# mjmyt/drone_path_planning_python

Hardware: AMD Instinct MI355X
Metric: minimum-snap trajectories/sec (N drones × M segments, order 7) at 1/2/4/8 MI355X (higher is better)
Workload: dtype f64

## Files before the change

### drone_path_planning_python_amd/csrc/msnap_collide.hip

```cpp
#include <math.h>

#include "msnap_internal.h"
#include "msnap_collide.h"
#include "msnap_wave.h"

namespace msnap {


struct CollideGeom {
  int R, ro, Cn, S;
  int Rp;
  int os, oe;
  int sym;
  int n_rb;
  int upw;
  int upw_tail;
  long long split;
  int sparts;
  long long total;
  long long u_lo, u_n;
  int I_lo, I_hi;
  int part;
};

// ... 395 lines not shown
        const int e = threadIdx.x + u * kSelThreads;
        bv[u] = e < nG * 6 ? cu.colbox[e] : 0.0;
      }
#pragma unroll
      for (int u = 0; u < kStageGroups * 6 / kSelThreads; ++u) {
        const int e = threadIdx.x + u * kSelThreads;
        if (e < nG * 6) sBox[e] = bv[u];
      }
    }
    __syncthreads();
  }
  auto load_box = [&](int gq, double(&B)[6]) {
#pragma unroll
    for (int k = 0; k < 6; ++k) {
      if constexpr (kStage) B[k] = sBox[gq * 6 + k];
      else B[k] = cu.colbox[(size_t)gq * 6 + k];
    }
  };
  if ((int)blockIdx.x >= n_rb) {
    constexpr int NW = kSelThreads / kWave, NS = kSelGroups * kSelTrips;
    __shared__ int gsum[NS * NW + 1];
    __shared__ int gbase, gtot;
    const int a0 = (blockIdx.x - n_rb) * kSelGroups, nG = (N + kColBlock - 1) / kColBlock;
    const int lane = threadIdx.x & (kWave - 1), w = threadIdx.x / kWave;
    unsigned long long kept = 0;
#pragma unroll
    for (int ai = 0; ai < kSelGroups; ++ai) {
      const int a = a0 + ai;
      double A[7], A6[6];
      load_box(a < nG ? a : nG - 1, A6);
#pragma unroll
      for (int k = 0; k < 6; ++k) A[k] = A6[k];
      A[6] = sCmax[a < nG ? a : nG - 1];
#pragma unroll
      for (int t = 0; t < kSelTrips; ++t) {
        bool keep = false;
        if (a + t * kSelThreads < nG) {
          const int b = a + t * kSelThreads + threadIdx.x, bc = b < nG ? b : nG - 1;
          double B6[6];
          load_box(bc, B6);
          const double lb2 = box_box_lb2(A, B6);
          keep = b < nG && (b == a || !((lb2 > A[6]) & (lb2 > sCmax[bc])));
        }
        const unsigned long long m = __ballot(keep);
        kept |= keep ? 1ull << (ai * kSelTrips + t) : 0ull;
        if (lane == 0) gsum[(ai * kSelTrips + t) * NW + w] = __popcll(m);
      }
    }
    __syncthreads();
    if (threadIdx.x < kWave) {
      int run = 0;
      for (int i0 = 0; i0 < NS * NW; i0 += kWave) {
        const int v = i0 + lane < NS * NW ? gsum[i0 + lane] : 0;
        int inc = v;
#pragma unroll
        for (int m = 1; m < kWave; m <<= 1) {
          const int o = __shfl_up(inc, m);
          inc += lane >= m ? o : 0;
        }
        if (i0 + lane < NS * NW) gsum[i0 + lane] = run + inc - v;
        run += __shfl(inc, kWave - 1);
      }
      if (lane == 0) {
        gbase = atomicAdd(&meta[kMetaGroups], run);
        gtot = run;
      }
    }
    __syncthreads();
    if (threadIdx.x < kSelGroups && a0 + (int)threadIdx.x < nG) {
      const int ai = threadIdx.x;
      const int s0 = gsum[ai * kSelTrips * NW], s1 = ai + 1 < kSelGroups ? gsum[(ai + 1) * kSelTrips * NW] : gtot;
      cg.astart[a0 + ai] = gbase + s0;
      cg.acnt[a0 + ai] = s1 - s0;
    }
#pragma unroll
    for (int ai = 0; ai < kSelGroups; ++ai)
#pragma unroll
      for (int t = 0; t < kSelTrips; ++t) {
        const bool keep = (kept >> (ai * kSelTrips + t)) & 1ull;
        const unsigned long long m = __ballot(keep);
        const int pos = gbase + gsum[(ai * kSelTrips + t) * NW + w] + __popcll(m & ((1ull << lane) - 1ull));
        if (keep && pos < cg.cap) {
          const int a = a0 + ai, b = a + t * kSelThreads + threadIdx.x;
          cg.glist[pos] = (a << 16) | b;
          if (b != a) cg.blist[(size_t)b * cg.nG + a] = pos + 1;
        }
      }
    return;
  }
  constexpr int GPB = kRowBlock / kColBlock;
  constexpr int NW = kSelThreads / kWave;
  __shared__ int wsum[kSelTrips][NW];
  __shared__ int sStart;
  __shared__ double sRow[GPB][8];
  __shared__ double sAll[8];
  const int I = blockIdx.x, lane = threadIdx.x & (kWave - 1), w = threadIdx.x / kWave;
  const int nsh = (N - I * kRowBlock + kColBlock - 1) / kColBlock;
  const int ng = nsh < GPB ? nsh : GPB;
  if (threadIdx.x < 7 * GPB) {
    const int q = threadIdx.x / 7, k = threadIdx.x % 7;
    if (q < ng) sRow[q][k] = k < 6 ? (kStage ? sBox[(I * GPB + q) * 6 + k] : cu.colbox[(size_t)(I * GPB + q) * 6 + k]) : sCmax[I * GPB + q];
  }
  __syncthreads();
  if (threadIdx.x < 7) {
    const int k = threadIdx.x;
    double v = sRow[0][k];
    for (int q = 1; q < ng; ++q) v = k < 3 ? fmin(v, sRow[q][k]) : fmax(v, sRow[q][k]);
    sAll[k] = v;
  }
  __syncthreads();
  unsigned long long mk[kSelTrips];
  bool keep[kSelTrips];
  double cbx[kSelTrips][6], cmx[kSelTrips];
#pragma unroll
  for (int t = 0; t < kSelTrips; ++t) {
    if (t * kSelThreads >= nsh) continue;
    const int k = t * kSelThreads + threadIdx.x, J = I * GPB + (k < nsh ? k : nsh - 1);
    load_box(J, cbx[t]);
    cmx[t] = sCmax[J];
  }
#pragma unroll
  for (int t = 0; t < kSelTrips; ++t) {
    const int k = t * kSelThreads + threadIdx.x;
    keep[t] = false;
    if (k < nsh) {
      keep[t] = true;
      if (k >= GPB) {
        const double cm = cmx[t];
        bool any = false;
        const double lb0 = box_box_lb2(sAll, cbx[t]);
        if (!((lb0 > sAll[6]) & (lb0 > cm))) {
          for (int q = 0; q < ng; ++q) {
            const double lb2 = box_box_lb2(sRow[q], cbx[t]);
            any |= !((lb2 > sRow[q][6]) & (lb2 > cm));
          }
        }
        keep[t] = any;
      }
    }
    mk[t] = __ballot(keep[t]);
    if (lane == 0) wsum[t][w] = __popcll(mk[t]);
  }
  __syncthreads();
  int all = 0, off[kSelTrips];
#pragma unroll
  for (int t = 0; t < kSelTrips; ++t) {
#pragma unroll
    for (int q = 0; q < NW; ++q) {
      if (q == w) off[t] = all;
      all += wsum[t][q];
    }
  }
  if (threadIdx.x == 0) {
    const int start = atomicAdd(&meta[kMetaTotal], all);
    sStart = start;
    meta[kMetaStart + I] = start;
    cnt[I] = all;
  }
  __syncthreads();
#pragma unroll
  for (int t = 0; t < kSelTrips; ++t)
    if (keep[t]) list[sStart + off[t] + __popcll(mk[t] & ((1ull << lane) - 1ull))] = (I << 16) | (t * kSelThreads + threadIdx.x);
}

__device__ __forceinline__ void
collide_span_list_body(const double *__restrict__ prow_t, const double *__restrict__ pcol, CollideGeom g,
                       double *__restrict__ part_d2, int32_t *__restrict__ part_j, double *__restrict__ cpart_d2,
                       int32_t *__restrict__ cpart_i, const int32_t *__restrict__ oid, const int32_t *__restrict__ list,
                       int sp_force, int slots, int32_t *__restrict__ meta) {
  constexpr int CB = kColBlock;
  __shared__ double sFold[CB * kWave];
  __shared__ int sFoldI[CB * kWave];
  const int lane = threadIdx.x;
  const int tot = meta[kMetaTotal];
  const CullSplit sp = cull_split(tot, slots, cull_nch(g.S), sp_force);
  if (blockIdx.x == 0 && lane == 0) {
    meta[kMetaParts] = sp.lo;
    meta[kMetaParts + 1] = sp.hi;
    meta[kMetaParts + 2] = sp.x;
  }
  const int items = sp.items(tot);
  const int xi = sp.x * sp.hi;
  auto share_of = [&](int it) { return it < xi ? it / sp.hi : sp.x + (it - xi) / sp.lo; };
  int it = blockIdx.x;
  int entry = it < items ? list[share_of(it)] : 0;
  while (it < items) {
    const int f = share_of(it);
    g.sparts = it < xi ? sp.hi : sp.lo;
    const int h = it - sp.item_of(f);
    const int I = entry >> 16, k = entry & 0xffff;
    const int nxt = it + gridDim.x;
    entry = nxt < items ? list[share_of(nxt)] : 0;
    const int crow = I * sp.hi + h;
    const int cj = I * kRowBlock + k * CB;
    const int ncols = g.Cn - cj < CB ? g.Cn - cj : CB;
    const bool two_sided = k >= kRowBlock / CB;
    RowSet rs;
#pragma unroll
    for (int rr = 0; rr < kRowsPerLane; ++rr) {
      const int raw = I * kRowBlock + rr * kWave + lane;
      rs.live[rr] = raw < g.R;
      rs.grow[rr] = rs.live[rr] ? raw : g.R - 1;
      rs.best[rr] = INFINITY;
      rs.bestj[rr] = -1;
    }
    const double *prowT = prow_t + (size_t)I * kRowBlock;
    if (ncols <= 2)
      collide_block<2, true>(g, prowT, pcol, cj, ncols, two_sided, rs, I, h, crow, lane, sFold, sFoldI, cpart_d2, cpart_i, oid);
    else if (ncols <= CB / 2)
      collide_block<CB / 2, true>(g, prowT, pcol, cj, ncols, two_sided, rs, I, h, crow, lane, sFold, sFoldI, cpart_d2, cpart_i, oid);
    else
      collide_block<CB, true>(g, prowT, pcol, cj, ncols, two_sided, rs, I, h, crow, lane, sFold, sFoldI, cpart_d2, cpart_i, oid);
#pragma unroll
    for (int rr = 0; rr < kRowsPerLane; ++rr) {
      part_d2[(size_t)it * kRowBlock + rr * kWave + lane] = rs.best[rr];
      part_j[(size_t)it * kRowBlock + rr * kWave + lane] = (rs.best[rr] == INFINITY) ? -1 : rs.bestj[rr];
    }
    it = nxt;
  }
}

constexpr int kGroupHalf = kColBlock / 2;
constexpr int kGroupLanes = kWave / 2;

constexpr int kFinishWaves = 4;
template <int kChunks>
__global__ void __launch_bounds__(kWave * kFinishWaves)
collide_finish_groups_kernel(int N, const int32_t *__restrict__ oid, const int32_t *__restrict__ meta, CullGroups cg,
                             double radius, double *__restrict__ min_dist, int32_t *__restrict__ partner,
                             int32_t *__restrict__ hit) {
  __shared__ int sItAll[kFinishWaves][kChunks * kWave];
  const int lane = threadIdx.x & (kWave - 1), w = __builtin_amdgcn_readfirstlane(threadIdx.x / kWave);
  int *sIt = sItAll[w];
  const int gq = blockIdx.x * kFinishWaves + w;
  if (gq >= cg.nG) return;
  int pl[kChunks];
#pragma unroll
  for (int c = 0; c < kChunks; ++c)
    pl[c] = (c * kWave < gq && c * kWave + lane < gq) ? cg.blist[(size_t)gq * cg.nG + c * kWave + lane] : 0;
  if (meta[kMetaGroups] > cg.cap) {
#pragma unroll
    for (int c = 0; c < kChunks; ++c)
      if (pl[c] > 0) cg.blist[(size_t)gq * cg.nG + c * kWave + lane] = 0;
    return;
  }
  const int nA = cg.acnt[gq], sA = cg.astart[gq];
  const int k = lane & (kColBlock - 1), e = lane >> 3;
  const int r = gq * kColBlock + k;
  const int out = r < N ? oid[r] : 0;
  int nB = 0;
#pragma unroll
  for (int c = 0; c < kChunks; ++c) {
    const unsigned long long m = __ballot(pl[c] > 0);
    if (pl[c] > 0) sIt[nB + __popcll(m & ((1ull << lane) - 1ull))] = pl[c] - 1;
    nB += __popcll(m);
  }
  __builtin_amdgcn_fence(__ATOMIC_RELEASE, "wavefront", "local");
  __builtin_amdgcn_wave_barrier();
  __builtin_amdgcn_fence(__ATOMIC_ACQUIRE, "wavefront", "local");
  double best = INFINITY;
  int bj = -1;
  constexpr int U = 8;
  for (int q0 = 0; q0 < nA + nB; q0 += U * (kWave / kColBlock)) {
    double d[U];
    int j[U];
#pragma unroll
    for (int u = 0; u < U; ++u) {
      const int q = q0 + u * (kWave / kColBlock) + e;
      d[u] = INFINITY;
      j[u] = -1;
      if (q < nA + nB) {
        const size_t slot = (q < nA ? (size_t)(sA + q) * 16 : (size_t)sIt[q - nA] * 16 + kColBlock) + k;
        d[u] = cg.cand_d2[slot];
        j[u] = cg.cand_j[slot];
      }
    }
#pragma unroll
    for (int u = 0; u < U; ++u)
      if (j[u] >= 0 && (bj < 0 || d[u] < best || (d[u] == best && j[u] < bj))) {
        best = d[u];
        bj = j[u];
      }
  }
#pragma unroll
  for (int m = kColBlock; m < kWave; m <<= 1) {
    const double o = shfl_xor_f64(best, m);
    const int oj = __shfl_xor(bj, m);
    if (oj >= 0 && (bj < 0 || o < best || (o == best && oj < bj))) {
      best = o;
      bj = oj;
    }
  }
  if (e == 0 && r < N) {
    const double dist = sqrt(bj >= 0 ? best : INFINITY);
    min_dist[out] = dist;
    partner[out] = bj;
    hit[out] = (dist < 2.0 * radius) ? 1 : 0;
  }
#pragma unroll
  for (int c = 0; c < kChunks; ++c)
    if (pl[c] > 0) cg.blist[(size_t)gq * cg.nG + c * kWave + lane] = 0;
}

constexpr int kGroupWaves = 4;
__global__ void __launch_bounds__(kWave, kGroupWaves)
collide_eval_groups_kernel(const double *__restrict__ pcol, int N, int S, const int32_t *__restrict__ oid,
                           const int32_t *__restrict__ meta, CullGroups cg, unsigned long long *__restrict__ hint) {
#pragma clang fp contract(off)
  const int lane = threadIdx.x;
  int tot = meta[kMetaGroups];
  if (blockIdx.x == 0 && lane == 0 && hint != nullptr)
    __hip_atomic_store(hint, cull_hint_pack(N, meta[kMetaTotal], tot), __ATOMIC_RELAXED, __HIP_MEMORY_SCOPE_SYSTEM);
  if (tot > cg.cap) tot = 0;
  const unsigned stride = (unsigned)S * 3u;
  const int per = (tot + 7) >> 3;
  auto item_of = [&](int v) { return (v >> 3) < per ? (v & 7) * per + (v >> 3) : tot; };
  int v = blockIdx.x, it = item_of(v);
  int entry = (it < tot && it < cg.cap) ? cg.glist[it] : 0;
  for (; (v >> 3) < per; v += gridDim.x, it = item_of(v)) {
    const int it_next = item_of(v + (int)gridDim.x);
    const int ent_raw = entry;
    entry = it_next < tot ? cg.glist[it_next] : 0;
    if (it >= tot) continue;
    const int ent = __builtin_amdgcn_readfirstlane(ent_raw);
    const int a = ent >> 16, b = ent & 0xffff;
    const bool diag = a == b;

    int lane_s = threadIdx.x;
    asm volatile("" : "+v"(lane_s));
    const int half = lane_s >> 5, ls = lane_s & (kGroupLanes - 1);
    double acc[kColBlock * kGroupHalf];
#pragma unroll
    for (int p = 0; p < kColBlock * kGroupHalf; ++p) acc[p] = INFINITY;
#pragma unroll 1
    for (int s0 = 0; s0 < S; s0 += kGroupLanes) {
      const int sq = s0 + ls < S ? s0 + ls : S - 1;
      const unsigned voff = (unsigned)sq * 24u;
      double cx[kGroupHalf], cy[kGroupHalf], cz[kGroupHalf];
#pragma unroll
      for (int c = 0; c < kGroupHalf; ++c) {
        const int d = b * kColBlock + half * kGroupHalf + c;
        const double *p = reinterpret_cast<const double *>(
            reinterpret_cast<const char *>(pcol + (size_t)(d < N ? d : N - 1) * stride) + (size_t)voff);
        cx[c] = p[0];
        cy[c] = p[1];
        cz[c] = p[2];
      }
      double rw[3][3];
      auto fetch = [&](int r, double(&dst)[3]) {
        const int d = a * kColBlock + r;
        const double *p = reinterpret_cast<const double *>(
            reinterpret_cast<const char *>(pcol + (size_t)(d < N ? d : N - 1) * stride) + (size_t)voff);
        dst[0] = p[0];
        dst[1] = p[1];
        dst[2] = p[2];
      };
      fetch(0, rw[0]);
      fetch(1, rw[1]);
#pragma unroll
      for (int r = 0; r < kColBlock; ++r) {
        if (r + 2 < kColBlock) fetch(r + 2, rw[(r + 2) % 3]);
        asm volatile("" ::: "memory");
        const double x = rw[r % 3][0], y = rw[r % 3][1], z = rw[r % 3][2];
#pragma unroll
        for (int c = 0; c < kGroupHalf; ++c) {
          const double dx = cx[c] - x, dy = cy[c] - y, dz = cz[c] - z;
          const double d2 = __builtin_fma(dz, dz, __builtin_fma(dy, dy, dx * dx));
          asm("v_min_f64 %0, %1, %0" : "+v"(acc[r * kGroupHalf + c]) : "v"(d2));
        }
      }
    }
#pragma unroll
    for (int n = 16, m = 16; n >= 1; n >>= 1, m >>= 1) {
      const bool up = (lane_s & m) != 0;
#pragma unroll
      for (int i = 0; i < n; ++i) {
        const double keep = up ? acc[i + n] : acc[i], send = up ? acc[i] : acc[i + n];
        acc[i] = __builtin_fmin(keep, __shfl_xor(send, m));
      }
    }
    double v = acc[0];
    int lane_c = threadIdx.x;
    asm volatile("" : "+v"(lane_c));
    const int pr = (lane_c & (kGroupLanes - 1)) >> 2, pc = lane_c & (kGroupHalf - 1), half_c = lane_c >> 5;
    const int ra = a * kColBlock + pr, cb = b * kColBlock + half_c * kGroupHalf + pc;
    const int oi = oid[ra < N ? ra : N - 1], oj = oid[cb < N ? cb : N - 1];
    if (ra >= N || cb >= N || (diag && ra == cb)) v = INFINITY;
    {
      double w = v;
      int wj = oj;
#pragma unroll
      for (int m = 1; m <= 32; m = (m == 2 ? 32 : m << 1)) {
        const double o = __shfl_xor(w, m);
        const int ojx = __shfl_xor(wj, m);
        const bool take = (o < w) | ((o == w) & (ojx < wj));
        w = take ? o : w;
        wj = take ? ojx : wj;
      }
      if ((lane & 35) == 0) {
        cg.cand_d2[(size_t)it * 16 + pr] = w;
        cg.cand_j[(size_t)it * 16 + pr] = w < INFINITY ? wj : -1;
      }
    }
    {
      double w = v;
      int wi = oi;
#pragma unroll
      for (int m = 4; m <= 16; m <<= 1) {
        const double o = __shfl_xor(w, m);
        const int oix = __shfl_xor(wi, m);
        const bool take = (o < w) | ((o == w) & (oix < wi));
        w = take ? o : w;
        wi = take ? oix : wi;
      }
      if ((lane_c & (kGroupLanes - 1)) < kGroupHalf) {
        const int k = kColBlock + half_c * kGroupHalf + pc;
        cg.cand_d2[(size_t)it * 16 + k] = w;
        cg.cand_j[(size_t)it * 16 + k] = (!diag && w < INFINITY) ? wi : -1;
      }
    }
  }
}

__global__ void __launch_bounds__(kWave, 4)
collide_eval_shares_kernel(const double *__restrict__ prow_t, const double *__restrict__ pcol, CollideGeom g,
                           double *__restrict__ part_d2, int32_t *__restrict__ part_j, double *__restrict__ cpart_d2,
                           int32_t *__restrict__ cpart_i, const int32_t *__restrict__ oid, const int32_t *__restrict__ list,
                           int sp_force, int slots, int32_t *__restrict__ meta, unsigned long long *__restrict__ hint,
                           int groups_cap) {
  if (groups_cap > 0 && meta[kMetaGroups] <= groups_cap) return;
  if (blockIdx.x == 0 && threadIdx.x == 0 && hint != nullptr)
    __hip_atomic_store(hint, cull_hint_pack(g.R, meta[kMetaTotal], meta[kMetaGroups]), __ATOMIC_RELAXED,
                       __HIP_MEMORY_SCOPE_SYSTEM);
  collide_span_list_body(prow_t, pcol, g, part_d2, part_j, cpart_d2, cpart_i, oid, list, sp_force, slots, meta);
}

__global__ void __launch_bounds__(kWave)
collide_short_kernel(const double *__restrict__ prow, const double *__restrict__ pcol, int R, int ro, int Cn, int S,
                     double radius, double *__restrict__ min_dist, int32_t *__restrict__ partner,
                     int32_t *__restrict__ hit, int raw) {
#pragma clang fp contract(off)
  const int r = blockIdx.x * kWave + threadIdx.x;
  if (r >= R) return;
  const int grow = ro + r;
  const double *pr = prow + (size_t)r * S * 3;
  double best = INFINITY;
  int bestj = -1;
  for (int j = 0; j < Cn; ++j) {
    const double *pc = pcol + (size_t)j * S * 3;
    double m = INFINITY;
    for (int sq = 0; sq < S; ++sq) {
      const double dx = pc[(size_t)sq * 3 + 0] - pr[(size_t)sq * 3 + 0];
      const double dy = pc[(size_t)sq * 3 + 1] - pr[(size_t)sq * 3 + 1];
      const double dz = pc[(size_t)sq * 3 + 2] - pr[(size_t)sq * 3 + 2];
      const double d2 = __builtin_fma(dz, dz, __builtin_fma(dy, dy, dx * dx));
      m = __builtin_fmin(d2, m);
    }
    if (j == grow) m = INFINITY;
    if (m < best) {
      best = m;
      bestj = j;
    }
  }
  if (raw) {
    min_dist[r] = best;
    partner[r] = (best == INFINITY) ? -1 : bestj;
    return;
  }
  const double dist = sqrt(best);
  min_dist[r] = dist;
  partner[r] = (best == INFINITY) ? -1 : bestj;
  hit[r] = (dist < 2.0 * radius) ? 1 : 0;
}

constexpr int kMergeRows = 16;
constexpr int kMergeParts = 16;
__global__ void __launch_bounds__(kMergeRows * kMergeParts)
collide_merge_kernel(const double *__restrict__ part_d2, const int32_t *__restrict__ part_j, CollideGeom g,
                     const double *__restrict__ cpart_d2, const int32_t *__restrict__ cpart_i, double radius,
                     double *__restrict__ min_dist, int32_t *__restrict__ partner, int32_t *__restrict__ hit,
                     const int32_t *__restrict__ oid, const int32_t *__restrict__ cnt, const int32_t *__restrict__ meta,
                     int groups_cap = 0) {
  if (groups_cap > 0 && meta[kMetaGroups] <= groups_cap) return;
  __shared__ double sD[kMergeParts][kMergeRows];
  __shared__ int sJ[kMergeParts][kMergeRows];
  const int lr = threadIdx.x & (kMergeRows - 1), q = threadIdx.x / kMergeRows;
  const int r_raw = blockIdx.x * kMergeRows + lr;
  const int r = r_raw < g.R ? r_raw : g.R - 1;
  const int out = oid ? oid[r] : r;
  double best = INFINITY;
  int bj = -1;
  constexpr int U = 8;
  auto sweep = [&](const double *pd, const int32_t *pj, size_t pitch, int n) {
    for (int s0 = q; s0 < n; s0 += U * kMergeParts) {
      double v[U];
      int j[U];
#pragma unroll
      for (int k = 0; k < U; ++k) {
        const int sidx = s0 + k * kMergeParts;
        const int sc = sidx < n ? sidx : n - 1;
        v[k] = pd[(size_t)sc * pitch];
        j[k] = sidx < n ? pj[(size_t)sc * pitch] : -1;
      }
#pragma unroll
      for (int k = 0; k < U; ++k) {
        if (j[k] >= 0 && (v[k] < best || (v[k] == best && j[k] < bj))) {
          best = v[k];
          bj = j[k];
        }
      }
    }
  };
  if (cnt) {
    const int I = __builtin_amdgcn_readfirstlane(r / kRowBlock);
    CullSplit sp;
    sp.lo = meta[kMetaParts];
    sp.hi = meta[kMetaParts + 1];
    sp.x = meta[kMetaParts + 2];
    const int f0 = meta[kMetaStart + I], first_item = sp.item_of(f0), n_items = sp.item_of(f0 + cnt[I]) - first_item;
    const size_t first = (size_t)first_item * kRowBlock + (r - I * kRowBlock);
    sweep(part_d2 + first, part_j + first, kRowBlock, n_items);
    if (I > 0) sweep(cpart_d2 + r, cpart_i + r, (size_t)g.R, I * sp.hi);
  } else if (g.total > 0) {
    const int I = r / kRowBlock;
    long long ua = collide_ustart(g, I), ub = collide_ustart(g, I + 1) - 1;
    ua = ua < g.u_lo ? g.u_lo : ua;
    ub = ub >= g.u_lo + g.u_n ? g.u_lo + g.u_n - 1 : ub;
    if (ub >= ua) {
      const long long wf = collide_share_of(g, ua), wl = collide_share_of(g, ub);
      const size_t first = ((size_t)wf + (I - g.I_lo)) * g.sparts * kRowBlock + (r - I * kRowBlock);
      sweep(part_d2 + first, part_j + first, kRowBlock, (int)(wl - wf + 1) * g.sparts);
    }
    const int Ib = I < g.I_hi + 1 ? I : g.I_hi + 1;
    if (g.sym && Ib > g.I_lo) sweep(cpart_d2 + r, cpart_i + r, (size_t)g.R, (Ib - g.I_lo) * g.sparts);
  }
  sD[q][lr] = best;
  sJ[q][lr] = bj;
  __syncthreads();
  if (q == 0 && r_raw < g.R) {
#pragma unroll
    for (int k = 1; k < kMergeParts; ++k) {
      const double v = sD[k][lr];
      const int j = sJ[k][lr];
      if (j >= 0 && (v < best || (v == best && j < bj))) {
        best = v;
        bj = j;
      }
    }
    if (g.part) {
      min_dist[r] = best;
      partner[r] = bj;
    } else {
      const double dist = sqrt(best);
      min_dist[out] = dist;
      partner[out] = bj;
      hit[out] = (dist < 2.0 * radius) ? 1 : 0;
    }
  }
}

__global__ void __launch_bounds__(256)
collide_finish_kernel(const unsigned char *__restrict__ parts, size_t part_stride, int n_parts, int N, int row_offset,
                      int n_rows, double radius, double *__restrict__ min_dist, int32_t *__restrict__ partner,
                      int32_t *__restrict__ hit) {
  const int i = blockIdx.x * 256 + threadIdx.x;
  if (i >= n_rows) return;
  const int r = row_offset + i;
  double best = INFINITY;
  int bj = -1;
  for (int p = 0; p < n_parts; ++p) {
    const unsigned char *base = parts + (size_t)p * part_stride;
    const double v = reinterpret_cast<const double *>(base)[r];
    const int j = reinterpret_cast<const int32_t *>(base + (size_t)N * sizeof(double))[r];
    if (j >= 0 && (v < best || (v == best && j < bj))) {
      best = v;
      bj = j;
    }
  }
  const double dist = sqrt(best);
  min_dist[i] = dist;
  partner[i] = bj;
  hit[i] = (dist < 2.0 * radius) ? 1 : 0;
}

__global__ void __launch_bounds__(256) collide_part_clear_kernel(double *__restrict__ d2, int32_t *__restrict__ pj, int N) {
  const int i = blockIdx.x * 256 + threadIdx.x;
  if (i < N) {
    d2[i] = INFINITY;
    pj[i] = -1;
  }
}


__global__ void __launch_bounds__(kWave * kKeyDrones)
collide_key_kernel(const double *__restrict__ pos, int N, int S, double *__restrict__ box, unsigned *__restrict__ key) {
  const int lane = threadIdx.x & (kWave - 1);
  const int d = blockIdx.x * kKeyDrones + __builtin_amdgcn_readfirstlane(threadIdx.x / kWave);
  if (d >= N) return;
  const double *p = pos + (size_t)d * S * 3;
  double lo[3] = {INFINITY, INFINITY, INFINITY}, hi[3] = {-INFINITY, -INFINITY, -INFINITY};
  const int E = S * 3;
  for (int e0 = 0; e0 < E; e0 += 3 * kWave) {
#pragma unroll
    for (int q = 0; q < 3; ++q) {
      const int e = e0 + q * kWave + lane;
      const double v = e < E ? p[e] : __builtin_nan("");
      const int k = (lane + q) % 3;
      if (__builtin_isfinite(v)) {
#pragma unroll
        for (int kk = 0; kk < 3; ++kk)
          if (k == kk) {
            lo[kk] = v < lo[kk] ? v : lo[kk];
            hi[kk] = v > hi[kk] ? v : hi[kk];
          }
      }
    }
  }
#pragma unroll
  for (int k = 0; k < 3; ++k) {
    lo[k] = uniform_f64(wave_minmax_f64<false>(lo[k]));
    hi[k] = uniform_f64(wave_minmax_f64<true>(hi[k]));
  }
  if (lane < 3) {
    box[(size_t)d * 6 + lane] = lane == 0 ? lo[0] : lane == 1 ? lo[1] : lo[2];
    box[(size_t)d * 6 + 3 + lane] = lane == 0 ? hi[0] : lane == 1 ? hi[1] : hi[2];
  }
  if (lane == 0) key[d] = drone_sort_key(lo, hi);
}

constexpr int kRankWaves = 16;
constexpr int kRankTile = 16;
template <int kRankKeys>
__global__ void __launch_bounds__(kWave * kRankWaves)
collide_rank_kernel(const unsigned *__restrict__ key, int N, int32_t *__restrict__ perm, const double *__restrict__ box,
                    unsigned long long *__restrict__ bound, int32_t *__restrict__ zero, int n_zero,
                    int32_t *__restrict__ meta) {
  __shared__ int cnt[kRankWaves][kRankTile];
  {
    const int gid = blockIdx.x * (kWave * kRankWaves) + threadIdx.x;
    uniform_for<int>(threadIdx.x, n_zero, gridDim.x * (kWave * kRankWaves), [&](int z) { zero[z] = 0; },
                     blockIdx.x * (kWave * kRankWaves));
    if (gid == 0) {
      meta[kMetaTotal] = 0;
      meta[kMetaGroups] = 0;
    }
  }
  const int lane = threadIdx.x & (kWave - 1), w = __builtin_amdgcn_readfirstlane(threadIdx.x / kWave);
  const int nq = (N + kRankWaves * kWave - 1) / (kRankWaves * kWave);
  const int i0 = blockIdx.x * kRankTile;
  unsigned kraw[kRankKeys];
#pragma unroll
  for (int q = 0; q < kRankKeys; ++q) {
    const int j = (w * nq + q) * kWave + lane;
    kraw[q] = key[(q < nq && j < N) ? j : 0];
  }
  const unsigned ktile = key[i0 + (lane & (kRankTile - 1)) < N ? i0 + (lane & (kRankTile - 1)) : N - 1];
  double bx[6] = {0.0, 0.0, 0.0, 0.0, 0.0, 0.0};
  if (threadIdx.x < kRankTile && i0 + (int)threadIdx.x < N) {
#pragma unroll
    for (int k = 0; k < 6; ++k) bx[k] = box[(size_t)(i0 + threadIdx.x) * 6 + k];
  }
  unsigned long long mine[kRankKeys];
#pragma unroll
  for (int q = 0; q < kRankKeys; ++q) {
    const int j = (w * nq + q) * kWave + lane;
    mine[q] = (q < nq && j < N) ? ((unsigned long long)kraw[q] << 32) | (unsigned)j : ~0ull;
  }
#pragma unroll
  for (int t = 0; t < kRankTile; ++t) {
    const int i = i0 + t < N ? i0 + t : N - 1;
    const unsigned long long ki = ((unsigned long long)(unsigned)__builtin_amdgcn_readlane((int)ktile, t) << 32) | (unsigned)i;
    int c = 0;
#pragma unroll
    for (int q = 0; q < kRankKeys; ++q)
      if (q < nq) c += __popcll(__ballot(mine[q] < ki));
    if (lane == 0) cnt[w][t] = c;
  }
  lds_barrier();
  if (threadIdx.x < kRankTile && i0 + (int)threadIdx.x < N) {
    int r = 0;
#pragma unroll
    for (int q = 0; q < kRankWaves; ++q) r += cnt[q][threadIdx.x];
    const int i = i0 + threadIdx.x;
    perm[r] = i;
    const bool has = (bx[0] <= bx[3]) & (bx[1] <= bx[4]) & (bx[2] <= bx[5]);
// ... 29 lines not shown
#pragma unroll
    for (int k = 0; k < 6; ++k) g6[k] = k < 3 ? INFINITY : -INFINITY;
    if (r < N) {
      const double *bx = box + (size_t)perm[r] * 6;
#pragma unroll
      for (int k = 0; k < 6; ++k) g6[k] = bx[k];
    }
#pragma unroll
    for (int k = 0; k < 6; ++k) {
      auto fold = [k](double a, double c) { return k < 3 ? fmin(a, c) : fmax(a, c); };
      g6[k] = fold(g6[k], dpp_f64<0xB1>(g6[k]));
      g6[k] = fold(g6[k], dpp_f64<0x4E>(g6[k]));
      g6[k] = fold(g6[k], dpp_f64<0x141>(g6[k]));
    }
    if ((tid & 7) == 0 && gq * kColBlock < N) {
#pragma unroll
      for (int k = 0; k < 6; ++k) colbox[(size_t)gq * 6 + k] = g6[k];
    }
    return;
  }
  const int bx = blockIdx.x % nx, by = blockIdx.x / nx;
  const int r0 = bx * kTileRows, e0 = by * kTileE;
  const int ne = E - e0 < kTileE ? E - e0 : kTileE;
  __shared__ int sPerm[kTileRows + kTileHalo];
  if (tid < kTileRows + kTileHalo) sPerm[tid] = perm[r0 + tid < N ? r0 + tid : N - 1];
  __syncthreads();
  constexpr int kElems = (kTileRows + kTileHalo) * kTileE, kPer = (kElems + 255) / 256;
  double val[kPer];
#pragma unroll
  for (int u = 0; u < kPer; ++u) {
    const int idx = tid + u * 256, i = idx / kTileE, tx = idx - i * kTileE;
    val[u] = (idx < kElems && tx < ne) ? pos[(size_t)sPerm[i] * E + e0 + tx] : 0.0;
  }
#pragma unroll
  for (int u = 0; u < kPer; ++u) {
    const int idx = tid + u * 256, i = idx / kTileE, tx = idx - i * kTileE;
    if (idx < kElems) {
      tile[i * kTilePitch + tx] = val[u];
      if (i < kTileRows && tx < ne && r0 + i < N) psorted[(size_t)(r0 + i) * E + e0 + tx] = val[u];
    }
  }
  lds_barrier();
  {
    const int tx = tid & 63, ty = tid >> 6;
    uniform_for<int>(ty, ne, 4, [&](int i) { prow_t[(size_t)(e0 + i) * Rp + r0 + tx] = tile[tx * kTilePitch + i]; });
  }
  {
    const int row = tid & 63, k = (tid >> 6) + 1;
    const double *pa = tile + row * kTilePitch, *pb = tile + (row + k) * kTilePitch;
    double f = INFINITY;
    for (int q = 0; q < ne; q += 3) {
      const double dx = pb[q] - pa[q], dy = pb[q + 1] - pa[q + 1], dz = pb[q + 2] - pa[q + 2];
      f = __builtin_fmin(__builtin_fma(dz, dz, __builtin_fma(dy, dy, dx * dx)), f);
    }
    sF[k - 1][row] = r0 + row + k < N ? f : INFINITY;
  }
  lds_barrier();
  if (tid < kTileRows + kTileHalo) {
    double b = INFINITY;
#pragma unroll
    for (int k = 1; k <= kTileHalo; ++k) {
      if (tid < kTileRows) b = __builtin_fmin(b, sF[k - 1][tid]);
      if (tid >= k && tid - k < kTileRows) b = __builtin_fmin(b, sF[k - 1][tid - k]);
    }
    if (b < INFINITY && r0 + tid < N) atomicMin(&bound[r0 + tid], (unsigned long long)__double_as_longlong(b));
  }
}

bool collide_counts_by_groups(const msnap_ctx *ctx, int n_drones, int shares_surviving, int group_pairs_surviving) {
  if (ctx->collide_cull_mode == 1) return false;
  if (n_drones > kCullGroupMaxDrones && 2LL * group_pairs_surviving > kGroupCapLarge) return false;
  if (ctx->collide_cull_mode == 2) return true;
  return cull_groups_cheaper(shares_surviving, group_pairs_surviving);
}

bool formation_collide_takes_broad_phase(const msnap_ctx *ctx, int n_rows, int row_offset, int n_cols, int n_samples,
                                         bool no_sym) {
  if (n_samples < kSampleChunk || n_rows != n_cols || row_offset != 0 || ctx->collide_no_cull || no_sym) return false;
  const int cull_min = ctx->collide_cull_min_drones > 0 ? ctx->collide_cull_min_drones : kCullMinDrones;
  return n_rows >= cull_min && n_rows >= 2 * kRowBlock && n_rows <= kCullMaxDrones;
}


int launch_collide_transpose(msnap_ctx *ctx, const double *pos, int n_rows, int Rp, int E, double *out, int32_t *fill,
                             size_t fill_n) {
  const int ny = (E + 31) / 32;
  MSNAP_LAUNCH(ctx, collide_transpose_kernel, dim3(Rp / 64, ny + (fill ? 4 : 0)), dim3(256), 0, pos, n_rows, Rp, E, out,
               ny, fill, fill_n, (const int32_t *)nullptr, (double *)nullptr);
  return MSNAP_OK;
}

int launch_collide_keys(msnap_ctx *ctx, const double *pos, int N, int S, double *box, unsigned *key) {
  MSNAP_LAUNCH(ctx, collide_key_kernel, dim3((N + kKeyDrones - 1) / kKeyDrones), dim3(kWave * kKeyDrones), 0, pos, N, S,
               box, key);
  return MSNAP_OK;
}

struct Carver {
  char *base;
  size_t off;
  template <class T>
  T *take(size_t n) {
    T *p = base ? reinterpret_cast<T *>(base + off) : nullptr;
    off += n * sizeof(T);
    return p;
  }
};

template <class Bufs, class Dims>
static int carve_collide_work(msnap_ctx *ctx, Bufs (*layout)(Carver &, const Dims &), const Dims &d, Bufs &b) {
  Carver sizing{nullptr, 0};
  layout(sizing, d);
  int rc = ensure(ctx, ctx->collide_work, sizing.off + 64);
  if (rc) return rc;
  Carver c{(char *)ctx->collide_work.p, 0};
  b = layout(c, d);
  return MSNAP_OK;
}

struct SpanDims {
  size_t t_entries, part_entries, centries;
};
struct SpanBufs {
  double *rows_t, *pd, *cd;
  int32_t *pj, *ci;
};
static SpanBufs span_layout(Carver &c, const SpanDims &d) {
  return SpanBufs{c.take<double>(d.t_entries),       c.take<double>(d.part_entries), c.take<double>(d.centries),
                  c.take<int32_t>(d.part_entries), c.take<int32_t>(d.centries)};
}

struct BroadDims {
  size_t Rp, E, N, nJ, entries, centries, gcap, shares, n_rb, blist_n;
};
struct BroadBufs {
  double *rows_t, *psorted, *box_own, *colbox;
  unsigned long long *bound;
  double *pd, *cd, *cand_d2;
  int32_t *pj, *ci;
  unsigned *key_own;
  int32_t *perm, *surv, *cnt, *meta, *acnt, *astart, *blist, *glist, *cand_j;
};
static BroadBufs broad_layout(Carver &c, const BroadDims &d) {
  return BroadBufs{c.take<double>(d.Rp * d.E), c.take<double>(d.N * d.E),  c.take<double>(d.N * 6),
                   c.take<double>(d.nJ * 6),   c.take<unsigned long long>(d.N),
                   c.take<double>(d.entries),  c.take<double>(d.centries), c.take<double>(d.gcap * 16),
                   c.take<int32_t>(d.entries), c.take<int32_t>(d.centries),
                   c.take<unsigned>(d.N),
                   c.take<int32_t>(d.N),       c.take<int32_t>(d.shares),  c.take<int32_t>(d.n_rb),
                   c.take<int32_t>(kMetaWords), c.take<int32_t>(d.nJ),     c.take<int32_t>(d.nJ),
                   c.take<int32_t>(d.blist_n), c.take<int32_t>(d.gcap),    c.take<int32_t>(d.gcap * 16)};
}

static int launch_span_merge(msnap_ctx *ctx, const CollideGeom &g, long long waves, const double *rows, int n_img_rows,
                             const double *rows_t_in, const double *pos_cols, const SpanBufs &b, size_t fill_n,
                             double radius, double *min_dist, int32_t *partner, int32_t *hit) {
  if (waves > 0) {
    if (!rows_t_in) {
      int rc = launch_collide_transpose(ctx, rows, n_img_rows, g.Rp, g.S * 3, b.rows_t, fill_n ? b.ci : nullptr, fill_n);
      if (rc) return rc;
    }
    MSNAP_LAUNCH(ctx, collide_span_kernel, dim3((unsigned)(waves * g.sparts)), dim3(kWave), 0,
                 rows_t_in ? rows_t_in : (const double *)b.rows_t, pos_cols, g, b.pd, b.pj, b.cd, b.ci);
  }
  MSNAP_LAUNCH(ctx, collide_merge_kernel, dim3((g.R + kMergeRows - 1) / kMergeRows), dim3(kMergeRows * kMergeParts), 0,
               (const double *)b.pd, (const int32_t *)b.pj, g, (const double *)b.cd, (const int32_t *)b.ci, radius,
               min_dist, partner, hit, (const int32_t *)nullptr, (const int32_t *)nullptr, (const int32_t *)nullptr);
  return MSNAP_OK;
}

struct WholePlan {
  long long upw;
  long long slots;
  long long waves;
  size_t cpart_entries;
  bool cull;
};

static WholePlan plan_whole_pass(const msnap_ctx *ctx, int n_rows, int row_offset, int n_cols, int n_samples,
                                 bool no_sym, CollideGeom &g) {
  WholePlan p{1, (long long)ctx->n_cu * 4 * 4, 0, 0, false};
  g.R = n_rows;
  g.ro = row_offset;
  g.Cn = n_cols;
  g.S = n_samples;
  g.n_rb = (n_rows + kRowBlock - 1) / kRowBlock;
  g.Rp = g.n_rb * kRowBlock;
  g.sparts = 1;
  g.u_lo = 0;
  g.u_n = 0;
  g.I_lo = 0;
  g.I_hi = g.n_rb - 1;
  g.part = 0;
  if (n_cols == 0) {
    g.os = g.oe = 0;
    g.sym = 0;
    g.upw = g.upw_tail = 1;
    g.split = 0;
    g.total = 0;
    return p;
  }
  const bool rows_in_cols = (long long)row_offset + n_rows <= n_cols;
  g.os = rows_in_cols ? row_offset : n_cols;
  g.oe = rows_in_cols ? row_offset + n_rows : n_cols;
  p.cpart_entries = (size_t)g.n_rb * n_rows;
  g.sym = (rows_in_cols && n_rows > kRowBlock && !no_sym && p.cpart_entries * 12 <= ((size_t)2 << 30)) ? 1 : 0;
  g.upw = 1;
  g.total = collide_ustart(g, g.n_rb);
  g.u_n = g.total;
  long long upw = kColBlock;
  const long long slots = p.slots;
  if (ctx->collide_waves_per_cu > 0) {
    upw = g.total / ((long long)ctx->n_cu * ctx->collide_waves_per_cu) / kColBlock * kColBlock;
    if (upw < kColBlock) upw = kColBlock;
  }
  while (((g.total + upw - 1) / upw + g.n_rb) * kRowBlock * 12 > ((long long)512 << 20)) upw *= 2;
  g.upw = (int)upw;
  g.upw_tail = (int)upw;
  g.split = (g.total + upw - 1) / upw * upw;
  const long long shares = (g.total + upw - 1) / upw;
  if (upw == kColBlock && ctx->collide_waves_per_cu == 0 && shares <= slots && n_rows == n_cols) {
    g.upw_tail = kColBlock / 2;
    g.split = shares * 3 / 4 * upw;
  } else if (upw == kColBlock && ctx->collide_waves_per_cu == 0 && shares % slots != 0 && shares % slots <= slots / 8) {
    g.upw_tail = 2;
    g.split = (shares - shares % slots) * upw;
  }
  p.upw = upw;
  p.waves = g.split / upw + (g.total - g.split + g.upw_tail - 1) / g.upw_tail;
  p.cull = g.sym && formation_collide_takes_broad_phase(ctx, n_rows, row_offset, n_cols, n_samples, no_sym);
  if (p.cull) return p;
  if (ctx->collide_sample_parts > 0) {
    g.sparts = ctx->collide_sample_parts < 8 ? ctx->collide_sample_parts : 8;
  } else if (ctx->collide_waves_per_cu == 0) {
    const int nch = (n_samples + kSampleChunk - 1) / kSampleChunk;
    while (g.sparts < 8 && p.waves * g.sparts < slots / 4 && nch / (g.sparts * 2) >= 2) g.sparts *= 2;
  }
  return p;
}

static int launch_broad_phase(msnap_ctx *ctx, const CollideGeom &g, long long slots, const double *pos_cols,
                              const double *rows_t_in, double radius, double *min_dist, int32_t *partner,
                              int32_t *hit) {
  const int N = g.R, n_samples = g.S, E = n_samples * 3;
  const size_t nJ = ((size_t)N + kColBlock - 1) / kColBlock;
  long long shares = 0;
  for (int I = 0; I < g.n_rb; ++I) shares += (N - I * kRowBlock + kColBlock - 1) / kColBlock;
  const long long all_groups = (long long)nJ * (nJ + 1) / 2;
  const bool all_fit = N <= kCullGroupMaxDrones;
  bool by_groups = false;
  if (ctx->collide_cull_mode == 2) {
    by_groups = true;
  } else if (ctx->collide_cull_mode != 1 && ctx->cull_hint) {
    const unsigned long long h = *(volatile unsigned long long *)ctx->cull_hint;
    const int hN = (int)(h >> 48) & 0x7fff;
    const long long hs = (long long)((h >> 24) & 0xffffff), hg = (long long)(h & 0xffffff);
    by_groups = h != 0 && hN == (N & 0x7fff) && hg != 0xffffff && cull_groups_cheaper(hs, hg) &&
                (all_fit || 2 * hg <= kGroupCapLarge);
  }
  const bool both = by_groups && !all_fit;
  const int spmax = N > 8192 ? 2 : kCullMaxParts;
  ctx->collide_last_shares = (int)shares;
  const int sp_force = (ctx->collide_sample_parts > 0 ? (ctx->collide_sample_parts < spmax ? ctx->collide_sample_parts : spmax) : 0) |
                       (spmax << 8);
  const long long items_max = (sp_force & 0xff) ? shares * (sp_force & 0xff) : (shares > 2 * slots ? shares : 2 * slots);
  const size_t entries = (by_groups && !both) ? 0 : (size_t)items_max * kRowBlock;
  const size_t centries = (by_groups && !both) ? 0 : (size_t)g.n_rb * spmax * N;
  const size_t gcap = !by_groups ? 0 : all_fit ? (size_t)all_groups : (size_t)kGroupCapLarge;
  const bool have_keys = handover_form(ctx, rows_t_in, pos_cols, N, n_samples) == 2;
  BroadBufs b;
  int rc = carve_collide_work(ctx, broad_layout,
                              BroadDims{(size_t)g.Rp, (size_t)E, (size_t)N, nJ, entries, centries, gcap, (size_t)shares,
                                        (size_t)g.n_rb, by_groups ? nJ * nJ : 0},
                              b);
  if (rc) return rc;
  const double *box = have_keys ? rows_t_in : b.box_own;
  const unsigned *key = have_keys ? reinterpret_cast<const unsigned *>(rows_t_in + (size_t)N * 6) : b.key_own;
  CullGroups cg{b.glist, b.astart, b.acnt, b.blist, b.cand_d2, b.cand_j, (int)gcap, (int)nJ};
  const bool trust = by_groups && !stream_is_capturing(ctx) && !ctx->collide_work.in_graph;
  const bool blist_clean = trust && ctx->blist_clean == (const void *)b.blist && ctx->blist_clean_n == (int)nJ;
  ctx->blist_clean = trust ? (const void *)b.blist : nullptr;
  ctx->blist_clean_n = (int)nJ;
  ctx->collide_meta = b.meta;
  ctx->collide_last_cull = 1;
  ctx->collide_last_by_groups = by_groups ? (all_fit ? 1 : 2) : 0;
  ctx->collide_last_n = N;
  ctx->collide_last_handover = have_keys ? 2 : 0;
  if (!have_keys) {
    rc = launch_collide_keys(ctx, pos_cols, N, n_samples, b.box_own, b.key_own);
    if (rc) return rc;
  }
  MSNAP_LAUNCH(ctx, (N <= 4096 ? collide_rank_kernel<4> : N <= 8192 ? collide_rank_kernel<8> : collide_rank_kernel<16>),
               dim3((N + kRankTile - 1) / kRankTile), dim3(kWave * kRankWaves), 0, key, N, b.perm, box, b.bound, b.blist,
               (int)(by_groups && !blist_clean ? nJ * nJ : 0), b.meta);
  const int nx = g.Rp / kTileRows, ny = (E + kTileE - 1) / kTileE;
  const int n_box = (int)((nJ + kBoxGroups - 1) / kBoxGroups), n_fill = centries ? 4 * nx : 0;
  MSNAP_LAUNCH(ctx, collide_gather_kernel, dim3((unsigned)(nx * ny + n_box + n_fill)), dim3(256), 0, pos_cols, N, g.Rp, E,
               b.rows_t, b.psorted, (const int32_t *)b.perm, b.bound, box, b.colbox, nx, ny, n_box, b.ci, centries);
  CollideCull cu{b.colbox};
  MSNAP_LAUNCH(ctx, (N <= kCullGroupMaxDrones ? collide_select_kernel<1> : collide_select_kernel<2>),
               dim3(g.n_rb + (unsigned)((nJ + kSelGroups - 1) / kSelGroups)), dim3(kSelThreads), 0, N, g.n_rb, cu,
               (const double *)b.bound, b.surv, b.cnt, b.meta, cg);
  if (by_groups) {
    MSNAP_LAUNCH(ctx, collide_eval_groups_kernel, dim3((unsigned)(ctx->n_cu * 4 * kGroupWaves)), dim3(kWave), 0,
                 (const double *)b.psorted, N, n_samples, (const int32_t *)b.perm, (const int32_t *)b.meta, cg,
                 ctx->cull_hint);
    MSNAP_LAUNCH(ctx, (N <= 4096 ? collide_finish_groups_kernel<8> : N <= 8192 ? collide_finish_groups_kernel<16> : collide_finish_groups_kernel<32>),
                 dim3((unsigned)((nJ + kFinishWaves - 1) / kFinishWaves)), dim3(kWave * kFinishWaves), 0, N,
                 (const int32_t *)b.perm, (const int32_t *)b.meta, cg, radius, min_dist, partner, hit);
    if (!both) return MSNAP_OK;
  }
  MSNAP_LAUNCH(ctx, collide_eval_shares_kernel, dim3((unsigned)slots), dim3(kWave), 0, (const double *)b.rows_t,
               (const double *)b.psorted, g, b.pd, b.pj, b.cd, b.ci, (const int32_t *)b.perm, (const int32_t *)b.surv,
               sp_force, (int)slots, b.meta, ctx->cull_hint, both ? (int)gcap : 0);
  MSNAP_LAUNCH(ctx, collide_merge_kernel, dim3((N + kMergeRows - 1) / kMergeRows), dim3(kMergeRows * kMergeParts), 0, b.pd,
               b.pj, g, b.cd, b.ci, radius, min_dist, partner, hit, (const int32_t *)b.perm, (const int32_t *)b.cnt,
               (const int32_t *)b.meta, both ? (int)gcap : 0);
  return MSNAP_OK;
}

int launch_formation_collide(msnap_ctx *ctx, int n_rows, int row_offset, int n_cols, int n_samples,
                             const double *pos_rows, const double *pos_cols, double radius, double *min_dist,
                             int32_t *partner, int32_t *hit, const double *rows_t_in, bool no_sym) {
  ctx->collide_last_handover = 0;
  if (n_cols > 0 && n_samples < kSampleChunk) {
    MSNAP_LAUNCH(ctx, collide_short_kernel, dim3((n_rows + kWave - 1) / kWave), dim3(kWave), 0, pos_rows, pos_cols,
                 n_rows, row_offset, n_cols, n_samples, radius, min_dist, partner, hit, 0);
    return MSNAP_OK;
  }
  CollideGeom g;
  const WholePlan p = plan_whole_pass(ctx, n_rows, row_offset, n_cols, n_samples, no_sym, g);
  if (n_cols == 0)
    return launch_span_merge(ctx, g, 0, nullptr, 0, nullptr, nullptr, SpanBufs{}, 0, radius, min_dist, partner, hit);
  ctx->collide_last_sym = g.sym;
  ctx->collide_last_cull = 0;
  ctx->collide_meta = nullptr;
  ctx->collide_last_shares = (int)(p.waves < 0x7fffffff ? p.waves : 0x7fffffff);
  if (p.cull) return launch_broad_phase(ctx, g, p.slots, pos_cols, rows_t_in, radius, min_dist, partner, hit);
  if (handover_form(ctx, rows_t_in, pos_rows, n_rows, n_samples) != 1) rows_t_in = nullptr;
  ctx->collide_last_handover = rows_t_in ? 1 : 0;
  if (p.upw > 0x3fffffff || p.waves * g.sparts > 0x7fffffff) return MSNAP_EINVAL;
  const size_t part_entries = ((size_t)p.waves + g.n_rb) * g.sparts * kRowBlock;
  const size_t centries = g.sym ? p.cpart_entries * g.sparts : 0;
  const size_t t_entries = rows_t_in ? 0 : (size_t)g.Rp * n_samples * 3;
  ctx->blist_clean = nullptr;
  SpanBufs b;
  int rc = carve_collide_work(ctx, span_layout, SpanDims{t_entries, part_entries, centries}, b);
  if (rc) return rc;
  return launch_span_merge(ctx, g, p.waves, pos_rows, n_rows, rows_t_in, pos_cols, b, 0, radius, min_dist, partner, hit);
}

static long long plan_part_pass(const msnap_ctx *ctx, int N, int n_samples, int part, int n_parts, CollideGeom &g,
                                int &nrb) {
  g.R = N;
  g.ro = 0;
  g.Cn = N;
  g.S = n_samples;
  g.n_rb = (N + kRowBlock - 1) / kRowBlock;
  g.os = 0;
  g.oe = N;
  g.sym = 1;
  g.total = collide_ustart(g, g.n_rb);
  auto cut = [&](int p) {
    const long long u = g.total * p / n_parts / kColBlock * kColBlock;
    return p >= n_parts ? g.total : u;
  };
  g.u_lo = cut(part);
  g.u_n = cut(part + 1) - g.u_lo;
  g.part = 1;
  g.sparts = 1;
  g.upw = g.upw_tail = kColBlock;
  g.I_lo = 0;
  g.I_hi = -1;
  const long long shares = (g.u_n + kColBlock - 1) / kColBlock;
  g.split = shares * kColBlock;
  long long waves = shares;
  if (shares > 0) {
    const long long u0 = g.u_lo, u1 = g.u_lo + g.u_n - 1;
    while (g.I_lo + 1 < g.n_rb && collide_ustart(g, g.I_lo + 1) <= u0) ++g.I_lo;
    g.I_hi = g.I_lo;
    while (g.I_hi + 1 < g.n_rb && collide_ustart(g, g.I_hi + 1) <= u1) ++g.I_hi;
    const long long slots = (long long)ctx->n_cu * 4 * 4;
    const int nch = (n_samples + kSampleChunk - 1) / kSampleChunk;
    if (ctx->collide_sample_parts > 0) {
      g.sparts = ctx->collide_sample_parts < 8 ? ctx->collide_sample_parts : 8;
    } else if (shares * 2 <= slots) {
      long long sp = slots / shares;
      sp = sp > 8 ? 8 : sp;
      while (sp > 1 && nch / sp < 2) --sp;
      g.sparts = (int)sp;
    } else if (shares % slots != 0 && shares % slots <= slots / 8 && shares > slots) {
      g.upw_tail = 2;
      g.split = (shares - shares % slots) * kColBlock;
    }
    waves = g.split / kColBlock + (g.u_n - g.split + g.upw_tail - 1) / g.upw_tail;
  }
  nrb = g.I_hi - g.I_lo + 1;
  g.Rp = (nrb > 0 ? nrb : 1) * kRowBlock;
  if (waves == 0) g.total = 0;
  return waves;
}

int launch_formation_collide_part(msnap_ctx *ctx, int N, int n_samples, const double *pos_all, int part, int n_parts,
                                  double *out_d2, int32_t *out_j) {
  if (n_samples < kSampleChunk) {
    const int r0 = (int)((long long)N * part / n_parts), r1 = (int)((long long)N * (part + 1) / n_parts);
    MSNAP_LAUNCH(ctx, collide_part_clear_kernel, dim3((N + 255) / 256), dim3(256), 0, out_d2, out_j, N);
    if (r1 > r0)
      MSNAP_LAUNCH(ctx, collide_short_kernel, dim3((r1 - r0 + kWave - 1) / kWave), dim3(kWave), 0,
                   pos_all + (size_t)r0 * n_samples * 3, pos_all, r1 - r0, r0, N, n_samples, 0.0, out_d2 + r0, out_j + r0,
                   (int32_t *)nullptr, 1);
    return MSNAP_OK;
  }
  CollideGeom g;
  int nrb;
  const long long waves = plan_part_pass(ctx, N, n_samples, part, n_parts, g, nrb);
  if (waves * g.sparts > 0x7fffffff) return MSNAP_EINVAL;
  const size_t part_entries = ((size_t)waves + (size_t)(nrb > 0 ? nrb : 0)) * g.sparts * kRowBlock;
  const size_t centries = (size_t)(nrb > 0 ? nrb : 0) * g.sparts * (size_t)N;
  const int E = n_samples * 3;
  const size_t t_entries = (size_t)g.Rp * E;
  if ((part_entries + centries) * 12 > ((size_t)16 << 30)) return MSNAP_ENOMEM;
  ctx->collide_last_cull = 0;
  ctx->collide_last_handover = 0;
  ctx->collide_meta = nullptr;
  ctx->blist_clean = nullptr;
  SpanBufs b;
  int rc = carve_collide_work(ctx, span_layout, SpanDims{t_entries, part_entries, centries}, b);
  if (rc) return rc;
  const int r_first = g.I_lo * kRowBlock;
  const int r_cnt = (N - r_first) < g.Rp ? (N - r_first) : g.Rp;
  return launch_span_merge(ctx, g, waves, pos_all + (size_t)r_first * E, r_cnt, nullptr, pos_all, b, centries, 0.0,
                           out_d2, out_j, nullptr);
}

int launch_formation_collide_finish(msnap_ctx *ctx, int N, int n_parts, const void *parts, size_t part_stride,
                                    int row_offset, int n_rows, double radius, double *min_dist, int32_t *partner,
                                    int32_t *hit) {
  MSNAP_LAUNCH(ctx, collide_finish_kernel, dim3((n_rows + 255) / 256), dim3(256), 0, (const unsigned char *)parts,
               part_stride, n_parts, N, row_offset, n_rows, radius, min_dist, partner, hit);
  return MSNAP_OK;
}

}
```

Before: 60.56 million.

## Share row-group positions across waves via double-buffered LDS staging in group eval

The group-eval kernel now launches one multi-wave block per row group `a` instead of a persistent grid of single-wave blocks walking the flat group list. Each wave takes one column group `b` from that row's contiguous slice of the list. The row group's sample positions are staged cooperatively into double-buffered shared memory, so the waves reuse one global load of the row data instead of each re-fetching it. In exchange it adds block-wide barriers each sample step, load imbalance when row groups have very different partner counts, and a dependence on per-row count and start arrays (`acnt`, `astart`) and on the list being grouped by row.

```diff
diff --git a/drone_path_planning_python_amd/csrc/msnap_collide.hip b/drone_path_planning_python_amd/csrc/msnap_collide.hip
--- a/drone_path_planning_python_amd/csrc/msnap_collide.hip
+++ b/drone_path_planning_python_amd/csrc/msnap_collide.hip
@@ -721,74 +721,106 @@
     if (pl[c] > 0) cg.blist[(size_t)gq * cg.nG + c * kWave + lane] = 0;
 }
 
-constexpr int kGroupWaves = 4;
-__global__ void __launch_bounds__(kWave, kGroupWaves)
+constexpr int kGroupWaves = 8;
+constexpr int kGroupChunk = kColBlock * kGroupLanes * 3;
+__device__ __host__ __forceinline__ unsigned group_eval_blocks(int nG) { return (unsigned)((nG + 7) / 8 * 8); }
+template <int W>
+__global__ void __launch_bounds__(kWave * W, 4)
 collide_eval_groups_kernel(const double *__restrict__ pcol, int N, int S, const int32_t *__restrict__ oid,
                            const int32_t *__restrict__ meta, CullGroups cg, unsigned long long *__restrict__ hint) {
 #pragma clang fp contract(off)
-  const int lane = threadIdx.x;
-  int tot = meta[kMetaGroups];
-  if (blockIdx.x == 0 && lane == 0 && hint != nullptr)
+  constexpr int NT = kWave * W;
+  constexpr int kStage = (kGroupChunk + NT - 1) / NT;
+  __shared__ double sRow[2][kGroupChunk];
+  const int lane = threadIdx.x & (kWave - 1), w = __builtin_amdgcn_readfirstlane(threadIdx.x / kWave);
+  const int tot = meta[kMetaGroups];
+  if (blockIdx.x == 0 && threadIdx.x == 0 && hint != nullptr)
     __hip_atomic_store(hint, cull_hint_pack(N, meta[kMetaTotal], tot), __ATOMIC_RELAXED, __HIP_MEMORY_SCOPE_SYSTEM);
-  if (tot > cg.cap) tot = 0;
+  if (tot > cg.cap) return;
+  const int per = gridDim.x >> 3;
+  const int a = (blockIdx.x & 7) * per + (blockIdx.x >> 3);
+  if (a >= cg.nG) return;
+  const int cnt = cg.acnt[a], first = cg.astart[a];
+  if (cnt <= 0) return;
   const unsigned stride = (unsigned)S * 3u;
-  const int per = (tot + 7) >> 3;
-  auto item_of = [&](int v) { return (v >> 3) < per ? (v & 7) * per + (v >> 3) : tot; };
-  int v = blockIdx.x, it = item_of(v);
-  int entry = (it < tot && it < cg.cap) ? cg.glist[it] : 0;
-  for (; (v >> 3) < per; v += gridDim.x, it = item_of(v)) {
-    const int it_next = item_of(v + (int)gridDim.x);
-    const int ent_raw = entry;
-    entry = it_next < tot ? cg.glist[it_next] : 0;
-    if (it >= tot) continue;
-    const int ent = __builtin_amdgcn_readfirstlane(ent_raw);
-    const int a = ent >> 16, b = ent & 0xffff;
+  const double *rows = pcol + (size_t)a * kColBlock * stride;
+  unsigned eoff[kStage];
+  int spos[kStage];
+#pragma unroll
+  for (int k = 0; k < kStage; ++k) {
+    const int e = threadIdx.x + k * NT, ec = e < kGroupChunk ? e : kGroupChunk - 1;
+    const int r = ec / (kGroupLanes * 3), o = ec - r * (kGroupLanes * 3);
+    const int rc = a * kColBlock + r < N ? r : N - 1 - a * kColBlock;
+    spos[k] = o / 3;
+    eoff[k] = (unsigned)rc * stride + (unsigned)(o - spos[k] * 3);
+  }
+  double st[kStage];
+  auto stage_load = [&](int s0) {
+#pragma unroll
+    for (int k = 0; k < kStage; ++k) {
+      const int sq = s0 + spos[k] < S ? s0 + spos[k] : S - 1;
+      st[k] = rows[eoff[k] + (unsigned)sq * 3u];
+    }
+  };
+  auto stage_store = [&](int buf) {
+#pragma unroll
+    for (int k = 0; k < kStage; ++k)
+      if ((int)threadIdx.x + k * NT < kGroupChunk) sRow[buf][threadIdx.x + k * NT] = st[k];
+  };
+  for (int q0 = 0; q0 < cnt; q0 += W) {
+    const bool active = q0 + w < cnt;
+    const int it = first + q0 + w;
+    const int ent = __builtin_amdgcn_readfirstlane(active ? cg.glist[it] : 0);
+    const int b = ent & 0xffff;
     const bool diag = a == b;
 
-    int lane_s = threadIdx.x;
+    int lane_s = lane;
     asm volatile("" : "+v"(lane_s));
     const int half = lane_s >> 5, ls = lane_s & (kGroupLanes - 1);
     double acc[kColBlock * kGroupHalf];
 #pragma unroll
     for (int p = 0; p < kColBlock * kGroupHalf; ++p) acc[p] = INFINITY;
+    int s_first = 0;
+    asm volatile("" : "+s"(s_first));
+    stage_load(s_first);
+    stage_store(0);
+    __syncthreads();
+    int buf = 0;
 #pragma unroll 1
-    for (int s0 = 0; s0 < S; s0 += kGroupLanes) {
-      const int sq = s0 + ls < S ? s0 + ls : S - 1;
-      const unsigned voff = (unsigned)sq * 24u;
+    for (int s0 = 0; s0 < S; s0 += kGroupLanes, buf ^= 1) {
+      const bool more = s0 + kGroupLanes < S;
       double cx[kGroupHalf], cy[kGroupHalf], cz[kGroupHalf];
-#pragma unroll
-      for (int c = 0; c < kGroupHalf; ++c) {
-        const int d = b * kColBlock + half * kGroupHalf + c;
-        const double *p = reinterpret_cast<const double *>(
-            reinterpret_cast<const char *>(pcol + (size_t)(d < N ? d : N - 1) * stride) + (size_t)voff);
-        cx[c] = p[0];
-        cy[c] = p[1];
-        cz[c] = p[2];
-      }
-      double rw[3][3];
-      auto fetch = [&](int r, double(&dst)[3]) {
-        const int d = a * kColBlock + r;
-        const double *p = reinterpret_cast<const double *>(
-            reinterpret_cast<const char *>(pcol + (size_t)(d < N ? d : N - 1) * stride) + (size_t)voff);
-        dst[0] = p[0];
-        dst[1] = p[1];
-        dst[2] = p[2];
-      };
-      fetch(0, rw[0]);
-      fetch(1, rw[1]);
-#pragma unroll
-      for (int r = 0; r < kColBlock; ++r) {
-        if (r + 2 < kColBlock) fetch(r + 2, rw[(r + 2) % 3]);
-        asm volatile("" ::: "memory");
-        const double x = rw[r % 3][0], y = rw[r % 3][1], z = rw[r % 3][2];
+      if (active) {
+        const int sq = s0 + ls < S ? s0 + ls : S - 1;
+        const unsigned voff = (unsigned)sq * 24u;
 #pragma unroll
         for (int c = 0; c < kGroupHalf; ++c) {
-          const double dx = cx[c] - x, dy = cy[c] - y, dz = cz[c] - z;
-          const double d2 = __builtin_fma(dz, dz, __builtin_fma(dy, dy, dx * dx));
-          asm("v_min_f64 %0, %1, %0" : "+v"(acc[r * kGroupHalf + c]) : "v"(d2));
+          const int d = b * kColBlock + half * kGroupHalf + c;
+          const double *p = reinterpret_cast<const double *>(
+              reinterpret_cast<const char *>(pcol + (size_t)(d < N ? d : N - 1) * stride) + (size_t)voff);
+          cx[c] = p[0];
+          cy[c] = p[1];
+          cz[c] = p[2];
         }
       }
-    }
+      if (more) stage_load(s0 + kGroupLanes);
+      if (active) {
+        const double *rowp = &sRow[buf][ls * 3];
+#pragma unroll
+        for (int r = 0; r < kColBlock; ++r) {
+          const double x = rowp[r * kGroupLanes * 3], y = rowp[r * kGroupLanes * 3 + 1], z = rowp[r * kGroupLanes * 3 + 2];
+#pragma unroll
+          for (int c = 0; c < kGroupHalf; ++c) {
+            const double dx = cx[c] - x, dy = cy[c] - y, dz = cz[c] - z;
+            const double d2 = __builtin_fma(dz, dz, __builtin_fma(dy, dy, dx * dx));
+            asm("v_min_f64 %0, %1, %0" : "+v"(acc[r * kGroupHalf + c]) : "v"(d2));
+          }
+        }
+      }
+      if (more) stage_store(buf ^ 1);
+      __syncthreads();
+    }
+    if (!active) continue;
 #pragma unroll
     for (int n = 16, m = 16; n >= 1; n >>= 1, m >>= 1) {
       const bool up = (lane_s & m) != 0;
@@ -799,7 +831,7 @@
       }
     }
     double v = acc[0];
-    int lane_c = threadIdx.x;
+    int lane_c = lane;
     asm volatile("" : "+v"(lane_c));
     const int pr = (lane_c & (kGroupLanes - 1)) >> 2, pc = lane_c & (kGroupHalf - 1), half_c = lane_c >> 5;
     const int ra = a * kColBlock + pr, cb = b * kColBlock + half_c * kGroupHalf + pc;
@@ -1435,7 +1467,7 @@
                dim3(g.n_rb + (unsigned)((nJ + kSelGroups - 1) / kSelGroups)), dim3(kSelThreads), 0, N, g.n_rb, cu,
                (const double *)b.bound, b.surv, b.cnt, b.meta, cg);
   if (by_groups) {
-    MSNAP_LAUNCH(ctx, collide_eval_groups_kernel, dim3((unsigned)(ctx->n_cu * 4 * kGroupWaves)), dim3(kWave), 0,
+    MSNAP_LAUNCH(ctx, collide_eval_groups_kernel<kGroupWaves>, dim3(group_eval_blocks((int)nJ)), dim3(kWave * kGroupWaves), 0,
                  (const double *)b.psorted, N, n_samples, (const int32_t *)b.perm, (const int32_t *)b.meta, cg,
                  ctx->cull_hint);
     MSNAP_LAUNCH(ctx, (N <= 4096 ? collide_finish_groups_kernel<8> : N <= 8192 ? collide_finish_groups_kernel<16> : collide_finish_groups_kernel<32>),
```

Measured after the change: 60.56 million (median of 2 runs). No clear change (+0.0%).
